# kekeliu-whu/Wildcat-SLAM

Measured on AMD Instinct MI355X. Metric: surfel-extract Mpts/s, higher is better.
Workload: dtype f64; 1 GPU; C2: 1M-pt single scan (G2 patch lattice, 999936 pts -> 31248 surfels) per GPU, voxel-grid + 3-level octree + per-cell 3x3 PCA; input = the reference's 48-byte hilti_ros::Point records, consumed in place; points_per_gpu=999936, surfels_per_gpu=31248, parallelism=sweep-per-gpu x1

## Files before the change

### wildcat-slam_amd/csrc/ctx.hip

```cpp
#include "ctx.h"

#include <cmath>
#include <cstring>
#include <mutex>

extern "C" const char *wc_version(void) { return "wildcat_hip 0.1 (gfx950)"; }

extern "C" int wc_device_count(void) {
  int n = 0;
  if (hipGetDeviceCount(&n) != hipSuccess) return 0;
  return n;
}

extern "C" void wc_params_default(wc_params *p) {
  std::memset(p, 0, sizeof(*p));
  p->voxel_size = 0.8f;
  p->max_layer = 2;
  p->min_points = 20;
  p->planer_threshold = 0.01f;
  p->min_plane_likeness = 0.1;
  p->cluster_gap = 0.05;
  p->cluster_min_points = 20;
  p->center_scale = 1.0;
  p->angular_scale = 5.0 * M_PI / 180.0;
// ... 37 lines not shown
    {"no_bucket_sort", "WC_NO_BUCKET_SORT", &wc_dev_opts::no_bucket_sort, true},
    {"ex_sync", "WC_EX_SYNC", &wc_dev_opts::ex_sync, true},
    {"match_pair_serial", "WC_MATCH_PAIR_SERIAL", &wc_dev_opts::match_pair_serial, true},
    {"lm_dense", "WC_LM_DENSE", &wc_dev_opts::lm_dense, true},
    {"lm_one_collective", "WC_LM_ONE_COLLECTIVE", &wc_dev_opts::lm_one_collective, true},
    {"lm_side_stream", "WC_LM_SIDE_STREAM", &wc_dev_opts::lm_side_stream, false},
    {"lm_dense_radius", "WC_LM_DENSE_RADIUS", &wc_dev_opts::lm_dense_radius, false},
    {"lm_radius0", "WC_LM_RADIUS0", &wc_dev_opts::lm_radius0, false},
};
}

namespace {
struct DevPool {
  hipMemPool_t pool = nullptr;
  int refs = 0;
};
std::mutex g_pool_mu;
DevPool g_pools[64];
}
hipMemPool_t wc_pool_acquire(int device) {
  if (device < 0 || device >= 64) return nullptr;
  std::lock_guard<std::mutex> lk(g_pool_mu);
  DevPool &d = g_pools[device];
  if (!d.pool) {
    int supported = 0;
    if (hipDeviceGetAttribute(&supported, hipDeviceAttributeMemoryPoolsSupported, device) != hipSuccess || !supported) {
      (void)hipGetLastError();
      return nullptr;
    }
    hipMemPoolProps props;
    std::memset(&props, 0, sizeof(props));
    props.allocType = hipMemAllocationTypePinned;
    props.handleTypes = hipMemHandleTypeNone;
    props.location.type = hipMemLocationTypeDevice;
    props.location.id = device;
    hipMemPool_t p = nullptr;
    if (hipMemPoolCreate(&p, &props) != hipSuccess || !p) {
      (void)hipGetLastError();
      return nullptr;
    }
    uint64_t keep = ~0ull;
    if (hipMemPoolSetAttribute(p, hipMemPoolAttrReleaseThreshold, &keep) != hipSuccess) (void)hipGetLastError();
    d.pool = p;
  }
  ++d.refs;
  return d.pool;
}
void wc_pool_release(int device, hipMemPool_t pool) {
  if (!pool || device < 0 || device >= 64) return;
  std::lock_guard<std::mutex> lk(g_pool_mu);
  DevPool &d = g_pools[device];
  if (d.pool == pool && --d.refs == 0) {
    (void)hipMemPoolDestroy(d.pool);
    d.pool = nullptr;
  }
}

extern "C" int wc_ctx_create(const wc_params *params, int device, wc_ctx **out) {
  if (!out) return WC_ERR_ARG;
  *out = nullptr;
  int n = 0;
  if (hipGetDeviceCount(&n) != hipSuccess || n <= 0 || device < 0 || device >= n) return WC_ERR_NOGPU;
  wc_ctx *ctx = new wc_ctx;
  ctx->device = device;
  if (params)
    ctx->P = *params;
  else
    wc_params_default(&ctx->P);
  int rc = check_params(ctx, &ctx->P);
  if (rc != WC_OK) {
    delete ctx;
    return rc;
  }
  int prev_dev = -1;
  (void)hipGetDevice(&prev_dev);
  struct Restore {
    int d;
    ~Restore() {
      if (d >= 0) (void)hipSetDevice(d);
    }
  } restore{prev_dev};
  if (hipSetDevice(device) != hipSuccess || hipStreamCreateWithFlags(&ctx->own_stream, hipStreamNonBlocking) != hipSuccess ||
      hipEventCreate(&ctx->ev0) != hipSuccess || hipEventCreate(&ctx->ev1) != hipSuccess ||
      hipHostMalloc((void **)&ctx->h_status, 128 * sizeof(uint32_t)) != hipSuccess ||
      hipHostMalloc((void **)&ctx->h_mail, (64 + 4096) * sizeof(double)) != hipSuccess) {
    delete ctx;
    return WC_ERR_HIP;
  }
  ctx->stream = ctx->own_stream;
  {
    void *dp = nullptr;
    if (hipHostGetDevicePointer(&dp, ctx->h_status, 0) == hipSuccess) ctx->h_status_dev = (uint32_t *)dp;
    for (int q = 0; q < 128; ++q) ctx->h_status[q] = 0;
  }
  for (wc_buf &b : ctx->b_route) b.plain = true;
  ctx->b_status.plain = true;
  ctx->pool = wc_pool_acquire(device);
  ctx->pool_ok = ctx->pool != nullptr;
#ifdef WC_DEV_KNOBS
  for (const DevOpt &o : kDevOpts)
    if (const char *v = getenv(o.env)) ctx->dev.*(o.field) = o.flag_only ? 1 : atoi(v);
#endif
  *out = ctx;
  return WC_OK;
}

extern "C" int wc_ctx_set_dev_option(wc_ctx *ctx, const char *name, int value) {
  if (!ctx || !name) return wc_fail(ctx, WC_ERR_ARG, "%s: null or out-of-range argument", __func__);
  for (const DevOpt &o : kDevOpts)
    if (strcmp(o.name, name) == 0) {
      ctx->dev.*(o.field) = value;
      ctx->ex.fx_backoff = ctx->ex.fx_skip_calls = 0;
      if (ctx->aux) ctx->aux->dev = ctx->dev;
      for (wc_ctx *sub : ctx->batch_subs) sub->dev = ctx->dev, sub->ex.fx_backoff = sub->ex.fx_skip_calls = 0;
      return WC_OK;
    }
  return wc_fail(ctx, WC_ERR_ARG, "wc_ctx_set_dev_option: unknown option '%s'", name);
}

void wc_window_free(wc_ctx *ctx);
extern "C" int wc_comm_rccl_destroy(wc_ctx *ctx);

extern "C" void wc_ctx_destroy(wc_ctx *ctx) {
  wc_dev_guard dg_(ctx);
  if (!ctx) return;
  (void)hipSetDevice(ctx->device);
  (void)hipStreamSynchronize(ctx->stream);
  if (ctx->pair_worker && ctx->pair_worker_free) ctx->pair_worker_free(ctx->pair_worker);
  ctx->pair_worker = nullptr;
  if (ctx->aux) {
    wc_ctx_destroy(ctx->aux);
    ctx->aux = nullptr;
  }
  if (ctx->ev_aux) (void)hipEventDestroy(ctx->ev_aux);
  if (ctx->ev_pair) (void)hipEventDestroy(ctx->ev_pair);
  for (hipEvent_t e : ctx->ev_knn)
    if (e) (void)hipEventDestroy(e);
  (void)wc_comm_rccl_destroy(ctx);
  wc_window_free(ctx);
  wc_buf *all[] = {&ctx->b_keys[0],      &ctx->b_keys[1],     &ctx->b_vals[0],     &ctx->b_vals[1],      &ctx->b_sorttmp,
                   &ctx->b_slots,        &ctx->b_slot_ids,    &ctx->b_slot_keys[0], &ctx->b_slot_keys[1], &ctx->b_slot_idx[0],
                   &ctx->b_slot_idx[1],  &ctx->b_cand,        &ctx->b_cand_meta,   &ctx->b_status,
                   &ctx->b_ex_ctrl};
  for (wc_buf *b : all) wc_buf_release(ctx, *b);
  for (wc_buf &b : ctx->b_misc) wc_buf_release(ctx, b);
  for (wc_buf &b : ctx->b_route) wc_buf_release(ctx, b);
  wc_buf_release(ctx, ctx->b_batch);
  for (wc_buf &b : ctx->b_kd) wc_buf_release(ctx, b);
  wc_buf_release(ctx, ctx->b_match_half);
  for (wc_ctx *sub : ctx->batch_subs) wc_ctx_destroy(sub);
  ctx->batch_subs.clear();
  for (wc_buf &b : ctx->b_fx) wc_buf_release(ctx, b);
  if (ctx->h_status) (void)hipHostFree(ctx->h_status);
  if (ctx->h_mail) (void)hipHostFree(ctx->h_mail);
  if (ctx->h_stage) (void)hipHostFree(ctx->h_stage);
  wc_buf_release(ctx, ctx->b_stage);
  (void)hipStreamSynchronize(ctx->stream);
  if (ctx->ev0) (void)hipEventDestroy(ctx->ev0);
  if (ctx->ev1) (void)hipEventDestroy(ctx->ev1);
  for (hipEvent_t e : ctx->ex_ev)
    if (e) (void)hipEventDestroy(e);
  if (ctx->own_stream) (void)hipStreamDestroy(ctx->own_stream);
  wc_pool_release(ctx->device, ctx->pool);
  delete ctx;
}

extern "C" const char *wc_last_error(const wc_ctx *ctx) { return ctx ? ctx->err.c_str() : "no context"; }
// ... 164 lines not shown
```

### wildcat-slam_amd/csrc/extract.hip

```cpp
#include <hip/hip_runtime.h>
#include <type_traits>

#include <chrono>
#include <cstdlib>
#include <cstring>
#include <rocprim/rocprim.hpp>

#include "ctx.h"
#include "dmath.h"

namespace {

constexpr int kMom = 11;
constexpr int kProdStride = 66;
constexpr unsigned kRootsGrid = 256 * 16;
constexpr unsigned kEmitGrid = 256 * 8;
constexpr unsigned kRoots2Grid = 256 * 4;
constexpr int kBuckets = 4096;
constexpr int kTile = 2048;
constexpr uint32_t kFlagKeyRange = 1u, kFlagSlotOverflow = 2u, kFlagTimeRange = 4u, kFlagBucketOverflow = 8u, kFlagSlotBinOverflow = 16u, kFlagLdsOverflow = 32u;

struct ExParams {
  double vs;
  float vs_f;
// ... 1120 lines not shown
      const uint32_t my_pos = (it + lane < it_end) ? A.heads[it + lane].pos : 0xFFFFFFFFu;
      unsigned long long live_mask = __ballot(my_pos != 0xFFFFFFFFu);
      while (live_mask) {
        uint32_t tslot = 0xFFFFFFFFu;
        for (int k = 0; k < NG; ++k) {
          if (!live_mask) break;
          const int bit = __ffsll((long long)live_mask) - 1;
          live_mask &= live_mask - 1;
          if (g == k) tslot = it + (uint32_t)bit;
        }
        do_roots(tslot);
      }
    }
  }
}

__global__ void __launch_bounds__(256) k_iota(uint32_t *v, uint64_t n) {
  const uint64_t i = (uint64_t)blockIdx.x * blockDim.x + threadIdx.x;
  if (i < n) v[i] = (uint32_t)i;
}

__global__ void __launch_bounds__(256) k_gather(const uint32_t *__restrict__ sorted_slot, const wc_surfel *__restrict__ slots,
                                               const wc_surfel_id *__restrict__ slot_ids, const uint32_t *status,
                                               wc_surfel *out, wc_surfel_id *out_ids, uint64_t cap) {
  if (status[1] & (kFlagBucketOverflow | kFlagKeyRange)) return;
  const uint64_t n = min((uint64_t)status[0], cap);
  const uint64_t i = (uint64_t)blockIdx.x * blockDim.x + threadIdx.x;
  const uint64_t rec = i / 10, part = i - rec * 10;
  if (rec >= n) return;
  const uint32_t s = sorted_slot[rec];
  if (part < 9) {
    const double2 *src = (const double2 *)(slots + s);
    double2 *dst = (double2 *)(out + rec);
    dst[part] = src[part];
  } else if (out_ids) {
    const uint4 *src = (const uint4 *)(slot_ids + s);
    uint4 *dst = (uint4 *)(out_ids + rec);
    *dst = *src;
  }
}

__device__ __forceinline__ bool surfel_id_less(const wc_surfel_id &a, const wc_surfel_id &b) {
  if (a.kx != b.kx) return a.kx < b.kx;
  if (a.ky != b.ky) return a.ky < b.ky;
  if (a.kz != b.kz) return a.kz < b.kz;
  return a.node < b.node;
}

__global__ void __launch_bounds__(256) k_fix_ties(const uint64_t *__restrict__ keys, uint32_t *idx, uint64_t n,
                                                 const wc_surfel_id *__restrict__ slot_ids) {
  const uint64_t i = (uint64_t)blockIdx.x * blockDim.x + threadIdx.x;
  if (i >= n) return;
  const uint64_t key = keys[i];
  if (key == ~0ull) return;
  if ((i > 0 && keys[i - 1] == key) || i + 1 >= n || keys[i + 1] != key) return;
  uint64_t e = i + 1;
  while (e < n && keys[e] == key) ++e;
  for (uint64_t a = i + 1; a < e; ++a) {
    const uint32_t v = idx[a];
    const wc_surfel_id vid = slot_ids[v];
    uint64_t b = a;
    while (b > i && surfel_id_less(vid, slot_ids[idx[b - 1]])) {
      idx[b] = idx[b - 1];
      --b;
    }
    idx[b] = v;
  }
}

constexpr int kSlotBinMax = 512;
struct SlotEmitArgs {
  const uint32_t *counts;
  const uint64_t *bins;
  uint32_t bin_cap;
  const wc_surfel *slots;
  const wc_surfel_id *slot_ids;
  uint32_t *status;
  wc_surfel *out;
  wc_surfel_id *out_ids;
  uint64_t cap;
  uint32_t *next_ctrl;
  uint32_t next_words;
};
__device__ __forceinline__ void slot_emit_body(const SlotEmitArgs &E, const uint32_t bid, const uint32_t nblk) {
  const uint32_t *__restrict__ counts = E.counts;
  const uint64_t *__restrict__ bins = E.bins;
  const uint32_t bin_cap = E.bin_cap;
  const wc_surfel *__restrict__ slots = E.slots;
  const wc_surfel_id *__restrict__ slot_ids = E.slot_ids;
  uint32_t *status = E.status;
  wc_surfel *out = E.out;
  wc_surfel_id *out_ids = E.out_ids;
  const uint64_t cap = E.cap;
  uint32_t *next_ctrl = E.next_ctrl;
  const uint32_t next_words = E.next_words;
  __shared__ uint64_t s_item[4][kSlotBinMax];
  if (next_ctrl) {
    const uint32_t i = bid * 256u + threadIdx.x;
    if (i < next_words) next_ctrl[i] = (i == 8u || i == 9u) ? status[i] : 0u;
  }
  __shared__ uint32_t s_sorted[4][kSlotBinMax];
  __shared__ uint32_t s_red[4];
  const int t = threadIdx.x, w = t >> 6, lane = t & 63;
  const uint32_t b0 = bid * 4u;
  static_assert(kBuckets / 4 <= 4 * 256, "four uint4 loads per thread cover the counts");
  const uint4 *c4 = (const uint4 *)counts;
  uint4 v[4];
#pragma unroll
  for (int k = 0; k < 4; ++k) {
    const uint32_t i = (uint32_t)t + 256u * k;
    v[k] = i < bid ? c4[i] : make_uint4(0u, 0u, 0u, 0u);
  }
  const uint4 own = c4[bid];
  const uint64_t *bin = bins + (size_t)(b0 + w) * bin_cap;
  const uint64_t first = (uint32_t)lane < bin_cap ? bin[lane] : 0ull;
  uint32_t part = 0;
#pragma unroll
  for (int k = 0; k < 4; ++k) part += v[k].x + v[k].y + v[k].z + v[k].w;
  for (int off = 32; off >= 1; off >>= 1) part += __shfl_xor(part, off);
  if (lane == 0) s_red[w] = part;
  __syncthreads();
  uint32_t base = s_red[0] + s_red[1] + s_red[2] + s_red[3];
  const uint32_t c0 = own.x, c1 = own.y, c2 = own.z, c3 = own.w;
  if (bid == nblk - 1 && t == 0) {
    status[0] = base + c0 + c1 + c2 + c3;
    uint32_t *hm = host_mailbox(status);
    if (hm) {
      hm[0] = base + c0 + c1 + c2 + c3;
      uint32_t queued = status[4];
      const uint32_t *fxc = counts + kBuckets;
      for (int j = 0; j < 16; ++j) queued += fxc[(16 + j) * 32];
      hm[4] = queued;
      hm[5] = status[5];
    }
  }
  base += (w > 0 ? c0 : 0u) + (w > 1 ? c1 : 0u) + (w > 2 ? c2 : 0u);
  const uint32_t c = w == 0 ? c0 : (w == 1 ? c1 : (w == 2 ? c2 : c3));
  if (c == 0) return;
  if (c > bin_cap) {
    if (lane == 0) raise_flag(status, kFlagSlotBinOverflow);
    return;
  }
  auto before = [&](uint64_t other, uint64_t mine) -> bool {
    if ((other >> 32) == (mine >> 32) && other != mine) {
      const double to = slots[(uint32_t)other].t, tm = slots[(uint32_t)mine].t;
      return to < tm || (to == tm && surfel_id_less(slot_ids[(uint32_t)other], slot_ids[(uint32_t)mine]));
    }
    return other < mine;
  };
  if (c <= 64u) {
    const uint32_t lo = (uint32_t)first, hi = (uint32_t)(first >> 32);
    uint32_t rank = 0;
    for (uint32_t j = 0; j < c; ++j) {
      const uint64_t other = ((uint64_t)(uint32_t)__builtin_amdgcn_readlane((int)hi, (int)j) << 32) | (uint32_t)__builtin_amdgcn_readlane((int)lo, (int)j);
      if ((uint32_t)lane < c) rank += before(other, first) ? 1u : 0u;
    }
    if ((uint32_t)lane < c) s_sorted[w][rank] = lo;
  } else {
    s_item[w][lane] = first;
    for (uint32_t i = lane + 64; i < c; i += 64) s_item[w][i] = bin[i];
    __builtin_amdgcn_wave_barrier();
    for (uint32_t i = lane; i < c; i += 64) {
      const uint64_t mine = s_item[w][i];
      uint32_t rank = 0;
      for (uint32_t j = 0; j < c; ++j) rank += before(s_item[w][j], mine) ? 1u : 0u;
      s_sorted[w][rank] = (uint32_t)mine;
    }
  }
  __builtin_amdgcn_wave_barrier();
  const int sub = lane / 10, piece = lane - sub * 10;
  if (sub >= 6) return;
  auto load = [&](uint32_t r, bool on) -> double2 {
    double2 d = make_double2(0.0, 0.0);
    if (!on) return d;
    const uint32_t sl = s_sorted[w][r];
    if (piece < 9)
      d = ((const double2 *)(slots + sl))[piece];
    else if (out_ids) {
      const uint4 q = *(const uint4 *)(slot_ids + sl);
      d = *(const double2 *)&q;
    }
    return d;
  };
  auto store = [&](uint32_t r, bool on, const double2 &d) {
    if (!on) return;
    const uint64_t o = (uint64_t)base + r;
    if (piece < 9)
      ((double2 *)(out + o))[piece] = d;
    else if (out_ids)
      *(double2 *)(out_ids + o) = d;
  };
  if (c <= 12u) {
    const uint32_t r = sub;
    const bool on0 = r < c && (uint64_t)base + r < cap, on1 = r + 6 < c && (uint64_t)base + r + 6 < cap;
    const double2 d0 = load(r, on0), d1 = load(r + 6, on1);
    store(r, on0, d0);
    store(r + 6, on1, d1);
    return;
  }
  for (uint32_t r = sub; r < c; r += 24) {
    bool on[4];
    double2 d[4];
#pragma unroll
    for (int q = 0; q < 4; ++q) {
      on[q] = r + 6u * q < c && (uint64_t)base + r + 6u * q < cap;
      d[q] = load(r + 6u * q, on[q]);
    }
#pragma unroll
    for (int q = 0; q < 4; ++q) store(r + 6u * q, on[q], d[q]);
  }
}

__global__ void __launch_bounds__(256) k_slot_emit(const uint32_t *__restrict__ counts, const uint64_t *__restrict__ bins, uint32_t bin_cap,
                                                  const wc_surfel *__restrict__ slots, const wc_surfel_id *__restrict__ slot_ids,
                                                  uint32_t *status, wc_surfel *out, wc_surfel_id *out_ids, uint64_t cap, uint32_t *next_ctrl,
                                                  uint32_t next_words) {
  const SlotEmitArgs E{counts, bins, bin_cap, slots, slot_ids, status, out, out_ids, cap, next_ctrl, next_words};
  slot_emit_body(E, blockIdx.x, gridDim.x);
}
__global__ void __launch_bounds__(256) k_slot_emit_b(const SlotEmitArgs *__restrict__ Es, int K) {
  const uint32_t per = kBuckets / 4;
  const uint32_t k = blockIdx.x / per;
  if ((int)k >= K) return;
  slot_emit_body(Es[k], blockIdx.x - k * per, per);
}


__device__ __forceinline__ uint32_t run_length(const unsigned long long *s_bits, uint32_t i, uint32_t cnt) {
  uint32_t w = (i + 1) >> 6;
  unsigned long long m = (w < kTile / 64) ? (s_bits[w] & (~0ull << ((i + 1) & 63))) : 0ull;
  while (m == 0ull && ++w < kTile / 64) m = s_bits[w];
  const uint32_t nxt = m ? (w * 64 + (uint32_t)__ffsll((long long)m) - 1) : cnt;
  return min(nxt, cnt) - i;
}

struct InitArgs {
  uint32_t *p[8];
  uint32_t nw[8];
  uint32_t val[8];
};
__global__ void __launch_bounds__(256) k_init(InitArgs I) {
  const uint32_t i = blockIdx.x * 256u + threadIdx.x;
#pragma unroll
  for (int r = 0; r < 8; ++r)
    if (i < I.nw[r]) I.p[r][i] = I.val[r];
}

constexpr int kRunThreads = 512;
__global__ void __launch_bounds__(kRunThreads) k_pt_runs(wc_points pts, double vs, uint64_t n, uint32_t *counts, uint64_t *bins,
                                                        uint32_t bin_cap, uint32_t *status) {
  __shared__ uint32_t s_key[kTile];
  __shared__ unsigned long long s_bits[kTile / 64];
  __shared__ uint32_t s_runs[kBuckets];
  __shared__ uint32_t s_pts[kBuckets];
  const int t = threadIdx.x;
  const uint64_t t0 = (uint64_t)blockIdx.x * kTile;
  const uint32_t cnt = (uint32_t)min((uint64_t)kTile, n - t0);
  double x0, y0, z0;
  load_xyz(pts, 0, x0, y0, z0);
  uint32_t key[kTile / kRunThreads];
#pragma unroll
  for (int j = 0; j < kTile / kRunThreads; ++j) {
    const uint32_t i = (uint32_t)j * kRunThreads + t;
    key[j] = 0;
    if (i < cnt) {
      double x, y, z;
      load_xyz(pts, t0 + i, x, y, z);
      int rx = vox(x, vs) - vox(x0, vs) + 512, ry = vox(y, vs) - vox(y0, vs) + 512, rz = vox(z, vs) - vox(z0, vs) + 512;
      if ((unsigned)rx >= 1024u || (unsigned)ry >= 1024u || (unsigned)rz >= 1024u) {
        raise_flag(status, kFlagKeyRange);
        rx = min(max(rx, 0), 1023), ry = min(max(ry, 0), 1023), rz = min(max(rz, 0), 1023);
      }
      key[j] = (uint32_t)rx | ((uint32_t)ry << 10) | ((uint32_t)rz << 20);
    }
  }
  for (int b = t; b < kBuckets; b += kRunThreads) {
    s_runs[b] = 0;
    s_pts[b] = 0;
  }
  if (t < kTile / 64) s_bits[t] = 0ull;
#pragma unroll
  for (int j = 0; j < kTile / kRunThreads; ++j) s_key[j * kRunThreads + t] = key[j];
  __syncthreads();
#pragma unroll
  for (int j = 0; j < kTile / kRunThreads; ++j) {
    const uint32_t i = (uint32_t)j * kRunThreads + t;
    const bool headp = i < cnt && (i == 0 || key[j] != s_key[i - 1]);
    const unsigned long long m = __ballot(headp);
    if ((t & 63) == 0) s_bits[i >> 6] = m;
  }
  __syncthreads();
  uint32_t rank[kTile / kRunThreads], len[kTile / kRunThreads];
#pragma unroll
  for (int j = 0; j < kTile / kRunThreads; ++j) {
    const uint32_t i = (uint32_t)j * kRunThreads + t;
    rank[j] = 0xFFFFFFFFu;
    if (i < cnt && ((s_bits[i >> 6] >> (i & 63)) & 1ull)) {
      const uint32_t d = key_digit(key[j]);
      len[j] = run_length(s_bits, i, cnt);
      rank[j] = atomicAdd(&s_runs[d], 1u);
      atomicAdd(&s_pts[d], len[j]);
    }
  }
  __syncthreads();
  for (int b = t; b < kBuckets; b += kRunThreads) {
    const uint32_t c = s_runs[b];
    if (c) {
// ... 53 lines not shown
    }
  } else {
    uint32_t N = 128;
    while (N < nb) N <<= 1;
    s_b[lane] = first;
    for (uint32_t i = lane + 64; i < N; i += 64) s_b[i] = (i < nb) ? bin[i] : ~0ull;
    __builtin_amdgcn_wave_barrier();
    for (uint32_t k = 2; k <= N; k <<= 1)
      for (uint32_t j = k >> 1; j > 0; j >>= 1) {
        for (uint32_t p = lane; p < N / 2; p += 64) {
          const uint32_t i = 2 * p - (p & (j - 1)), l = i + j;
          const uint64_t x = s_b[i], y = s_b[l];
          if ((x > y) == ((i & k) == 0)) {
            s_b[i] = y;
            s_b[l] = x;
          }
        }
        __builtin_amdgcn_wave_barrier();
      }
  }
  __builtin_amdgcn_wave_barrier();
  uint32_t carry = 0;
  for (uint32_t i0 = 0; i0 < nb; i0 += 64) {
    const uint32_t i = i0 + lane;
    const uint64_t c = (i < nb) ? s_b[i] : 0ull;
    const uint32_t l = (i < nb) ? comp_len(c) : 0u;
    uint32_t inc = l;
    for (int off = 1; off < 64; off <<= 1) {
      const uint32_t v = __shfl_up(inc, off);
      if (lane >= off) inc += v;
    }
    if (i < nb) {
      s_off[i] = carry + inc - l;
      bin[i] = c;
      run_off[(size_t)b * bin_cap + i] = carry + inc - l;
    }
    carry += __shfl(inc, 63);
  }
  __builtin_amdgcn_wave_barrier();
  uint32_t *s_list = (uint32_t *)s_a;
  uint32_t nlive = 0, next_head = nb;
  for (int i0 = (int)((nb + 63) / 64) * 64 - 64; i0 >= 0; i0 -= 64) {
    const uint32_t r = (uint32_t)i0 + lane;
    const bool in = r < nb;
    const uint32_t rest = in ? comp_rest(s_b[r]) : 0u;
    const bool head = in && (r == 0 || comp_rest(s_b[r - 1]) != rest);
    const unsigned long long hm = __ballot(head);
    const unsigned long long above = (lane == 63) ? 0ull : (hm >> (lane + 1));
    const uint32_t r2 = above ? r + (uint32_t)__ffsll((long long)above) : next_head;
    const uint32_t seg = (r2 < nb ? s_off[min(r2, nb - 1)] : total) - (in ? s_off[r] : 0u);
    const bool live = head && seg > (uint32_t)min_points;
    const unsigned long long lm = __ballot(live);
    if (live) s_list[nlive + (uint32_t)__popcll(lm & ((1ull << lane) - 1ull))] = r | (r2 << 16);
    nlive += (uint32_t)__popcll(lm);
    if (hm) next_head = (uint32_t)i0 + (uint32_t)__ffsll((long long)hm) - 1u;
  }
  if (lane == 0) s_live[w] = nlive;
  __syncthreads();
  const uint32_t pbase0 = s_red[0] + s_red[1] + s_red[2] + s_red[3];
  const uint32_t pbase = pbase0 + before;
  const uint32_t first_slot = pbase0 / (uint32_t)(min_points + 1);
  uint32_t lbase = 0;
  for (int j = 0; j < w; ++j) lbase += s_live[j];
  if (t == 0) {
    root_cnt[blockIdx.x] = s_live[0] + s_live[1] + s_live[2] + s_live[3];
    root_first[blockIdx.x] = first_slot;
  }
  for (uint32_t k = lane; k < nlive; k += 64) {
    const uint32_t r = s_list[k] & 0xFFFFu, r2 = s_list[k] >> 16;
    const uint32_t seg = (r2 < nb ? s_off[r2] : total) - s_off[r];
    head_slots[first_slot + lbase + k] = HeadRec{pbase + s_off[r], b * bin_cap + r, r2 - r, seg};
  }
}

constexpr uint32_t kPtBinMax = 1024;

inline uint32_t pt_bin_cap(uint64_t n) {
  uint32_t cap = 64;
  while (cap < kPtBinMax && (uint64_t)cap * kBuckets < 32 * n) cap *= 2;
  return cap;
}

constexpr uint32_t kCtrlStatus = 0, kCtrlCounts = 64, kCtrlRoots = kCtrlCounts + 2 * kBuckets, kCtrlBins = kCtrlRoots + 2 * (kBuckets / 4),
                   kCtrlFx = kCtrlBins + kBuckets, kCtrlWords = kCtrlFx + 4 * 16 * 32;

int clear_ctrl(wc_ctx *ctx) {
  WC_TRY(wc_ensure(ctx, ctx->b_ex_ctrl, kCtrlWords * 4));
  uint32_t *ctrl = (uint32_t *)ctx->b_ex_ctrl.p;
  InitArgs I{};
  void *dp = nullptr;
  if (hipHostGetDevicePointer(&dp, ctx->h_status, 0) != hipSuccess) dp = nullptr;
  const unsigned long long a = (unsigned long long)dp;
  I.p[0] = ctrl, I.nw[0] = 8, I.val[0] = 0u;
  I.p[1] = ctrl + 10, I.nw[1] = kCtrlRoots - 10, I.val[1] = 0u;
  I.p[2] = ctrl + 8, I.nw[2] = 1, I.val[2] = (uint32_t)a;
  I.p[3] = ctrl + 9, I.nw[3] = 1, I.val[3] = (uint32_t)(a >> 32);
  I.p[4] = ctrl + kCtrlBins, I.nw[4] = kBuckets + 4 * 16 * 32, I.val[4] = 0u;
  k_init<<<(kCtrlRoots + 255) / 256, 256, 0, ctx->stream>>>(I);
  WC_HIP(ctx, hipGetLastError());
  return WC_OK;
}

int point_sort_runs(wc_ctx *ctx, const wc_points &pts, double vs, HeadRec *head_slots, int min_points, uint32_t *status) {
  hipStream_t st = ctx->stream;
  const uint64_t n = pts.n;
  const uint32_t cap = pt_bin_cap(n);
  const uint32_t lds_cap = std::min(cap, std::max(64u, ctx->ex.lds_cap));
  WC_TRY(wc_ensure(ctx, ctx->b_misc[1], (uint64_t)kBuckets * cap * 8));
  WC_TRY(wc_ensure(ctx, ctx->b_misc[3], (uint64_t)kBuckets * cap * 4));
  uint32_t *counts = (uint32_t *)ctx->b_ex_ctrl.p + kCtrlCounts;
  const unsigned tiles = (unsigned)((n + kTile - 1) / kTile);
  const size_t lds = (size_t)4 * lds_cap * 20;
  if (!ctx->ex.bucket_attr_set) {
    WC_HIP(ctx, hipFuncSetAttribute((const void *)k_pt_bucket, hipFuncAttributeMaxDynamicSharedMemorySize, (int)(4 * kPtBinMax * 20)));
    ctx->ex.bucket_attr_set = true;
  }
  k_pt_runs<<<tiles, kRunThreads, 0, st>>>(pts, vs, n, counts, (uint64_t *)ctx->b_misc[1].p, cap, status);
  k_pt_bucket<<<kBuckets / 4, 256, lds, st>>>((uint64_t *)ctx->b_misc[1].p, cap, lds_cap, counts, (uint32_t *)ctx->b_misc[3].p, head_slots,
                                             counts + 2 * kBuckets, counts + 2 * kBuckets + kBuckets / 4, min_points, status);
  WC_HIP(ctx, hipGetLastError());
  return WC_OK;
}

template <typename K>
int sort_pairs(wc_ctx *ctx, K *kin, K *kout, uint32_t *vin, uint32_t *vout, size_t n, unsigned end_bit) {
  using cfg = rocprim::radix_sort_config<rocprim::default_config, rocprim::default_config, rocprim::default_config, 0>;
  size_t tmp = 0;
  WC_HIP(ctx, rocprim::radix_sort_pairs<cfg>(nullptr, tmp, kin, kout, vin, vout, n, 0u, end_bit, ctx->stream));
  WC_TRY(wc_ensure(ctx, ctx->b_sorttmp, tmp));
  tmp = ctx->b_sorttmp.cap;
  WC_HIP(ctx, rocprim::radix_sort_pairs<cfg>(ctx->b_sorttmp.p, tmp, kin, kout, vin, vout, n, 0u, end_bit, ctx->stream));
  return WC_OK;
}

#include "extract_fast.inc"
#include "extract_split.inc"

int fx_ensure_zero(wc_ctx *ctx, wc_buf &b, size_t bytes) {
  if (bytes <= b.cap) return WC_OK;
  WC_TRY(wc_ensure(ctx, b, bytes));
  WC_HIP(ctx, hipMemsetAsync(b.p, 0, b.cap, ctx->stream));
  return WC_OK;
}

bool fx_applicable(const wc_ctx *ctx, uint64_t n, double t_lo, double t_hi) {
  const wc_params &P = ctx->P;
  if (P.exact_sums || ctx->dev.exact_sums) return false;
  if (n < 64 || !(P.voxel_size > 0.0f) || P.voxel_size >= 0.99f) return false;
  if (!(P.cluster_gap > 1e-6) || !(t_hi > t_lo)) return false;
  if ((t_hi - t_lo) / (P.cluster_gap * 0.999) >= 1048000.0) return false;
  return true;
}

int fx_tail(wc_ctx *ctx, bool layer2);

int run_pipeline_fast(wc_ctx *ctx, const wc_points &pts, double t_lo, double t_hi, wc_surfel *d_out, wc_surfel_id *d_ids, uint64_t cap) {
  const wc_params &P = ctx->P;
  const uint64_t n = pts.n;
  hipStream_t st = ctx->stream;
  FxArgs A;
  std::memset(&A, 0, sizeof(A));
  ExParams &E = A.P;
  E.vs = (double)P.voxel_size, E.vs_f = P.voxel_size, E.max_layer = P.max_layer, E.min_points = P.min_points;
  E.thr = (double)P.planer_threshold, E.min_like = P.min_plane_likeness;
  for (int i = 0; i < 3; ++i) E.view[i] = P.view_point[i];
  E.gap = P.cluster_gap, E.cluster_min = P.cluster_min_points;
  E.t_lo_bits = ordered_bits_host(t_lo);
// ... 57 lines not shown
    ctx->ex.fx_dirty = false;
  }
  WC_TRY(wc_ensure(ctx, ctx->b_fx[5], (size_t)2 * kCtrlWords * 4));
  if (!ctx->ex.fx_ctrl_ready) {
    WC_HIP(ctx, hipMemsetAsync(ctx->b_fx[5].p, 0, (size_t)2 * kCtrlWords * 4, st));
    void *dp = nullptr;
    if (hipHostGetDevicePointer(&dp, ctx->h_status, 0) != hipSuccess) dp = nullptr;
    const unsigned long long a = (unsigned long long)dp;
    const uint32_t addr[2] = {(uint32_t)a, (uint32_t)(a >> 32)};
    for (int b = 0; b < 2; ++b)
      WC_HIP(ctx, hipMemcpyAsync((uint32_t *)ctx->b_fx[5].p + (size_t)b * kCtrlWords + 8, addr, 8, hipMemcpyHostToDevice, st));
    WC_HIP(ctx, hipStreamSynchronize(st));
    ctx->ex.fx_ctrl_ready = true;
    ctx->ex.fx_parity = 0;
  }
  uint32_t *ctrl = (uint32_t *)ctx->b_fx[5].p + (size_t)ctx->ex.fx_parity * kCtrlWords;
  for (int q = 0; q < 64; ++q) ctx->h_status[q] = 0;
  A.rkey = (uint32_t *)ctx->b_fx[0].p, A.rlist = (uint32_t *)ctx->b_fx[1].p;
  A.blk = (unsigned long long *)ctx->b_fx[2].p, A.blk2 = (unsigned long long *)ctx->b_fx[3].p;
  A.rec = (unsigned long long *)ctx->b_fx[4].p;
  A.jobs = (unsigned long long *)ctx->b_fx[6].p;
  A.status = ctrl + kCtrlStatus;
  A.cnt = ctrl + kCtrlFx;
  A.slots = (wc_surfel *)ctx->b_slots.p, A.slot_ids = (wc_surfel_id *)ctx->b_slot_ids.p;
  A.slots_per = (uint32_t)std::min<uint64_t>(total_slots / kFxSub, 0x7FFFFFFFu);
  A.slot_counts = ctrl + kCtrlBins;
  A.slot_bins = (uint64_t *)ctx->b_slot_keys[1].p;
  A.slot_bin_cap = bin_cap;
  auto mark = [&](int i) {
    if (ctx->ex_prof && (ctx->ex_prof_mode != 2 || i == 1 || i == 5)) (void)hipEventRecord(ctx->ex_ev[i], st);
  };
  mark(0);
  mark(1);
  static const bool dbg = wc_log_env("WC_FX_DEBUG");
  auto dbg_sync = [&](const char *what) {
    if (!dbg) return;
    fprintf(stderr, "[fx] %s ...", what);
    const hipError_t e = hipStreamSynchronize(st);
    uint32_t w[64], c[4 * 16 * 32];
    (void)hipMemcpy(w, A.status, sizeof(w), hipMemcpyDeviceToHost);
    (void)hipMemcpy(c, A.cnt, sizeof(c), hipMemcpyDeviceToHost);
    uint32_t r = 0, q = 0, sl = 0, sp = 0;
    for (int j = 0; j < 16; ++j) r += c[j * 32], q += c[(16 + j) * 32], sl += c[(32 + j) * 32], sp += c[(48 + j) * 32];
    fprintf(stderr, " %s flags=%u roots=%u nodes2=%u slots=%u spill=%u\n", hipGetErrorString(e), w[1], r, q, sl, sp);
  };
  if (dbg) fprintf(stderr, "[fx] n=%llu tiles=%u mr_per=%u mq_per=%u tr=%u slots_per=%u bin_cap=%u\n", (unsigned long long)n, tiles, A.mr_per, A.mq_per, tr, A.slots_per, bin_cap);
  if (ctx->ex.batch_defer) {
    static_assert(sizeof(FxArgs) <= sizeof(ctx->ex.roots_args), "ctx.h: roots_args too small");
    std::memcpy(ctx->ex.roots_args, &A, sizeof(A));
    ctx->ex.total_slots = total_slots;
    ctx->ex.bin_cap = bin_cap;
    ctx->ex.fast_slots = true;
    ctx->ex.tail = &fx_tail;
    ctx->ex.d_out = d_out, ctx->ex.d_ids = d_ids, ctx->ex.cap = cap;
    ctx->ex.layer2_done = P.max_layer >= 2 && ctx->ex.last_splits > 0;
    ctx->ex.fx_tiles = tiles, ctx->ex.fx_ngrid = std::max(64u, ngrid / 8u);
    ctx->ex.deferred = true;
    return WC_OK;
  }
  k_fx_acc<1><<<tiles, kFxThreads, 0, st>>>(A);
  dbg_sync("k_fx_acc<1>");
  mark(2);
  if (ctx->ex.fx_long_lists) k_fx_merge<1><<<std::min<unsigned>(ngrid * 2u, 8192u), 128, 0, st>>>(A);
  if (ctx->ex.fx_split) {
    k_fx_walk<1><<<ngrid, 64, 0, st>>>(A);
    dbg_sync("k_fx_walk<1>");
    k_fx_test<1><<<ngrid, 64, 0, st>>>(A);
  } else {
    k_fx_nodes<1><<<ngrid, 64, 0, st>>>(A);
  }
  dbg_sync("k_fx_nodes<1>");
  mark(3);
  static_assert(sizeof(FxArgs) <= sizeof(ctx->ex.roots_args), "ctx.h: roots_args too small");
  std::memcpy(ctx->ex.roots_args, &A, sizeof(A));
  ctx->ex.total_slots = total_slots;
  ctx->ex.bin_cap = bin_cap;
  ctx->ex.fast_slots = true;
  ctx->ex.tail = &fx_tail;
  ctx->ex.d_out = d_out, ctx->ex.d_ids = d_ids, ctx->ex.cap = cap;
  return fx_tail(ctx, P.max_layer >= 2 && ctx->ex.last_splits > 0);
}

constexpr int kMailTicket = 120;
__global__ void k_ex_ticket(uint32_t *host_word, uint32_t ticket) {
  __hip_atomic_store(host_word, ticket, __ATOMIC_RELEASE, __HIP_MEMORY_SCOPE_SYSTEM);
}

int fx_tail(wc_ctx *ctx, bool layer2) {
  hipStream_t st = ctx->stream;
  FxArgs A;
  std::memcpy(&A, ctx->ex.roots_args, sizeof(A));
  auto mark = [&](int i) {
    if (ctx->ex_prof && (ctx->ex_prof_mode != 2 || i == 1 || i == 5)) (void)hipEventRecord(ctx->ex_ev[i], st);
  };
  if (layer2) {
    const unsigned tiles = (unsigned)((A.pts.n + kFxTile - 1) / kFxTile);
    k_fx_acc<2><<<tiles, kFxThreads, 0, st>>>(A);
    const unsigned ngrid = std::min<unsigned>(256 * 16, std::max<unsigned>(64, (unsigned)(A.pts.n / 256)));
    if (ctx->ex.fx_long_lists2) k_fx_merge<2><<<std::min(8192u, std::max(64u, ctx->ex.last_splits)), 128, 0, st>>>(A);
    const unsigned g2 = std::min(std::min(256u * 8u, ngrid), std::max(64u, ctx->ex.last_splits));
    if (ctx->ex.fx_split) {
      k_fx_walk<2><<<g2, 64, 0, st>>>(A);
      k_fx_test<2><<<g2, 64, 0, st>>>(A);
    } else {
      k_fx_nodes<2><<<g2, 64, 0, st>>>(A);
    }
  }
  ctx->ex.layer2_done = layer2;
  mark(4);
  uint32_t *next_ctrl = (uint32_t *)ctx->b_fx[5].p + (size_t)(ctx->ex.fx_parity ^ 1) * kCtrlWords;
  static_assert(kCtrlWords <= (kBuckets / 4) * 256, "k_slot_emit's grid covers the control block");
  k_slot_emit<<<kBuckets / 4, 256, 0, st>>>(A.slot_counts, A.slot_bins, ctx->ex.bin_cap, (const wc_surfel *)ctx->b_slots.p,
                                           (const wc_surfel_id *)ctx->b_slot_ids.p, A.status, ctx->ex.d_out, ctx->ex.d_ids, ctx->ex.cap, next_ctrl,
                                           kCtrlWords);
  mark(5);
  ctx->ex.ticket = 0;
  if (ctx->h_status_dev && !ctx->ex_prof && !ctx->dev.ex_sync) {
    if (++ctx->ex.ticket_seq == 0u) ++ctx->ex.ticket_seq;
    ctx->ex.ticket = ctx->ex.ticket_seq;
    k_ex_ticket<<<1, 1, 0, st>>>(ctx->h_status_dev + kMailTicket, ctx->ex.ticket);
  }
  static const bool fx_dbg = wc_log_env("WC_FX_DEBUG");
  if (fx_dbg) fprintf(stderr, "[fx] k_slot_emit (layer2=%d) ... %s\n", (int)layer2, hipGetErrorString(hipStreamSynchronize(st)));
  WC_HIP(ctx, hipGetLastError());
  return WC_OK;
}

template <typename K, bool RUNS>
int pipeline_tail(wc_ctx *ctx, bool layer2) {
  hipStream_t st = ctx->stream;
  RootsArgs A;
  memcpy(&A, ctx->ex.roots_args, sizeof(A));
  uint32_t *status = A.status;
  wc_surfel *d_out = ctx->ex.d_out;
  wc_surfel_id *d_ids = ctx->ex.d_ids;
  const uint64_t cap = ctx->ex.cap, total_slots = ctx->ex.total_slots;
  auto mark = [&](int i) {
    if (ctx->ex_prof && (ctx->ex_prof_mode != 2 || i == 1 || i == 5)) (void)hipEventRecord(ctx->ex_ev[i], st);
  };
  if (layer2) {
    const unsigned grid2 = std::min(kRoots2Grid, std::max(64u, ctx->ex.last_splits));
    if constexpr (RUNS) {
      if (ctx->ex.unordered)
        k_roots_banks<K, 2, true><<<grid2, 64, 0, st>>>(A, (const K *)ctx->b_keys[1].p);
      else
        k_roots<K, 2, true><<<grid2, 64, 0, st>>>(A, (const K *)ctx->b_keys[1].p);
    } else {
      k_roots_banks<K, 2, false><<<grid2, 64, 0, st>>>(A, (const K *)ctx->b_keys[1].p);
    }
  }
  ctx->ex.layer2_done = layer2;
  mark(4);
  if (ctx->ex.fast_slots) {
    k_slot_emit<<<kBuckets / 4, 256, 0, st>>>((const uint32_t *)ctx->b_ex_ctrl.p + kCtrlBins, A.slot_bins, ctx->ex.bin_cap, (const wc_surfel *)ctx->b_slots.p,
                                             (const wc_surfel_id *)ctx->b_slot_ids.p, status, d_out, d_ids, cap, nullptr, 0u);
  } else {
    k_iota<<<(unsigned)((total_slots + 255) / 256), 256, 0, st>>>((uint32_t *)ctx->b_slot_idx[0].p, total_slots);
    WC_TRY(sort_pairs<uint64_t>(ctx, (uint64_t *)ctx->b_slot_keys[0].p, (uint64_t *)ctx->b_slot_keys[1].p,
                                (uint32_t *)ctx->b_slot_idx[0].p, (uint32_t *)ctx->b_slot_idx[1].p, total_slots,
                                ctx->ex.slot_end_bit));
    k_fix_ties<<<(unsigned)((total_slots + 255) / 256), 256, 0, st>>>((const uint64_t *)ctx->b_slot_keys[1].p, (uint32_t *)ctx->b_slot_idx[1].p,
                                                                     total_slots, (const wc_surfel_id *)ctx->b_slot_ids.p);
    const uint64_t gth = std::min<uint64_t>(total_slots, cap) * 10;
    if (gth)
      k_gather<<<(unsigned)((gth + 255) / 256), 256, 0, st>>>((const uint32_t *)ctx->b_slot_idx[1].p, (const wc_surfel *)ctx->b_slots.p,
                                                             (const wc_surfel_id *)ctx->b_slot_ids.p, status, d_out, d_ids, cap);
  }
  mark(5);
  if (!ctx->ex.fast_slots) WC_HIP(ctx, hipMemcpyAsync(ctx->h_status, status, 32, hipMemcpyDeviceToHost, st));
  WC_HIP(ctx, hipGetLastError());
  return WC_OK;
}

template <typename K>
int run_pipeline(wc_ctx *ctx, const wc_points &pts, double t_lo, double t_hi, wc_surfel *d_out, wc_surfel_id *d_ids,
                 uint64_t cap, bool fast, bool fast_order) {
  const wc_params &P = ctx->P;
  const uint64_t n = pts.n;
  hipStream_t st = ctx->stream;
  ExParams E;
  E.vs = (double)P.voxel_size;
  E.vs_f = P.voxel_size;
  E.max_layer = P.max_layer;
  E.min_points = P.min_points;
  E.thr = (double)P.planer_threshold;
  E.min_like = P.min_plane_likeness;
  for (int i = 0; i < 3; ++i) E.view[i] = P.view_point[i];
  E.gap = P.cluster_gap;
  E.cluster_min = P.cluster_min_points;
  E.t_lo_bits = ordered_bits_host(t_lo);
  E.dbg = ctx->dev.debug_skip;
  E.merge_min = ctx->dev.fx_merge_min;
  const uint64_t span = ordered_bits_host(t_hi) - E.t_lo_bits;
  E.t_span_bits = span;
  unsigned tbits = 1;
  while (tbits < 64 && (span >> tbits)) ++tbits;
  const unsigned slot_end_bit = tbits >= 63 ? 64 : tbits + 1;

  const uint64_t total_slots = (n * (uint64_t)(P.max_layer + 1)) / (uint64_t)P.cluster_min_points + 1;
  WC_TRY(wc_ensure(ctx, ctx->b_keys[0], n * sizeof(K)));
  WC_TRY(wc_ensure(ctx, ctx->b_keys[1], n * sizeof(K)));
  WC_TRY(wc_ensure(ctx, ctx->b_vals[0], n * 4));
  WC_TRY(wc_ensure(ctx, ctx->b_vals[1], n * 4));
  WC_TRY(wc_ensure(ctx, ctx->b_cand, total_slots * kMom * 8));
  WC_TRY(wc_ensure(ctx, ctx->b_cand_meta, total_slots * 4));
  WC_TRY(wc_ensure(ctx, ctx->b_slots, total_slots * sizeof(wc_surfel)));
  WC_TRY(wc_ensure(ctx, ctx->b_slot_ids, total_slots * sizeof(wc_surfel_id)));
  WC_TRY(wc_ensure(ctx, ctx->b_slot_keys[0], total_slots * 8));
  WC_TRY(wc_ensure(ctx, ctx->b_slot_keys[1], total_slots * 8));
  WC_TRY(wc_ensure(ctx, ctx->b_slot_idx[0], total_slots * 4));
  WC_TRY(wc_ensure(ctx, ctx->b_slot_idx[1], total_slots * 4));
  WC_TRY(wc_ensure(ctx, ctx->b_misc[0], (n / (uint64_t)(P.min_points + 1) + 2) * sizeof(HeadRec)));
  const bool precleared = ctx->ex.precleared && ctx->b_ex_ctrl.p;
  ctx->ex.precleared = false;
  if (!precleared) WC_TRY(clear_ctrl(ctx));
  for (int q = 0; q < 16; ++q) ctx->h_status[q] = 0;
  uint32_t *status = (uint32_t *)ctx->b_ex_ctrl.p + kCtrlStatus;

  auto mark = [&](int i) {
    if (ctx->ex_prof && (ctx->ex_prof_mode != 2 || i == 1 || i == 5)) (void)hipEventRecord(ctx->ex_ev[i], st);
  };
  mark(0);
  const bool fast_slots = fast_order && tbits <= 31 && total_slots < (1ull << 31);
  uint32_t bin_cap = 64;
  while (bin_cap < kSlotBinMax && (uint64_t)bin_cap * kBuckets < 2 * total_slots) bin_cap *= 2;
  const unsigned g256 = (unsigned)((n + 255) / 256);
  const bool fast_pts = fast && sizeof(K) == 4;
  if (fast_pts || fast_slots) {
    WC_TRY(wc_ensure(ctx, ctx->b_slot_keys[1], (uint64_t)kBuckets * bin_cap * 8));
  }
  const uint32_t nslots = (uint32_t)(n / (uint64_t)(P.min_points + 1) + 1);
  if (!fast_slots || !fast_pts) {
    InitArgs I{};
    int r = 0;
    auto fill = [&](void *p, uint64_t words, uint32_t v) { I.p[r] = (uint32_t *)p, I.nw[r] = (uint32_t)words, I.val[r] = v, ++r; };
    if (!fast_slots) fill(ctx->b_slot_keys[0].p, total_slots * 2, 0xFFFFFFFFu);
    if (!fast_pts) fill(ctx->b_misc[0].p, (uint64_t)nslots * 4, 0xFFFFFFFFu);
    uint32_t mx = 0;
// ... 395 lines not shown
```

Baseline: 21650 Mpts/s.

## Fold completion ticket into slot-emit via last-block arrival counters

Removes the separate single-thread ticket kernel launched after k_slot_emit. Each workgroup now counts itself on hierarchical arrival counters, and the last one publishes the host-visible ticket. Output stores go through buffer-resource b128 stores, and mailbox writes become system-scope atomics so the host can poll completion without an extra kernel launch. The cost is extra atomics per workgroup, a coherent host allocation for the status words, and added memory-ordering complexity: the publishes are relaxed atomics placed after a vmcnt wait.

Result: no change. 21370 Mpts/s, median of 2 (-1.3%).

```diff
diff --git a/wildcat-slam_amd/csrc/ctx.hip b/wildcat-slam_amd/csrc/ctx.hip
--- a/wildcat-slam_amd/csrc/ctx.hip
+++ b/wildcat-slam_amd/csrc/ctx.hip
@@ -143,7 +143,7 @@
   } restore{prev_dev};
   if (hipSetDevice(device) != hipSuccess || hipStreamCreateWithFlags(&ctx->own_stream, hipStreamNonBlocking) != hipSuccess ||
       hipEventCreate(&ctx->ev0) != hipSuccess || hipEventCreate(&ctx->ev1) != hipSuccess ||
-      hipHostMalloc((void **)&ctx->h_status, 128 * sizeof(uint32_t)) != hipSuccess ||
+      hipHostMalloc((void **)&ctx->h_status, 128 * sizeof(uint32_t), hipHostMallocCoherent) != hipSuccess ||
       hipHostMalloc((void **)&ctx->h_mail, (64 + 4096) * sizeof(double)) != hipSuccess) {
     delete ctx;
     return WC_ERR_HIP;
diff --git a/wildcat-slam_amd/csrc/extract.hip b/wildcat-slam_amd/csrc/extract.hip
--- a/wildcat-slam_amd/csrc/extract.hip
+++ b/wildcat-slam_amd/csrc/extract.hip
@@ -1226,9 +1226,32 @@
   uint32_t *next_ctrl;
   uint32_t next_words;
 };
-__device__ __forceinline__ void slot_emit_body(const SlotEmitArgs &E, const uint32_t bid, const uint32_t nblk) {
-  const uint32_t *__restrict__ counts = E.counts;
-  const uint64_t *__restrict__ bins = E.bins;
+constexpr uint32_t kArriveSubs = 32, kArriveWords = (kArriveSubs + 1) * 32;
+static_assert((kBuckets / 4) % kArriveSubs == 0, "every sub-counter counts the same number of workgroups");
+typedef __attribute__((address_space(1))) uint32_t gu32;
+struct SlotPublish {
+  uint32_t *arrive;
+  uint32_t *ticket_word;
+  uint32_t ticket;
+};
+
+__device__ __forceinline__ __amdgpu_buffer_rsrc_t wave_rsrc(const void *p) {
+  const unsigned long long a = (unsigned long long)p;
+  const unsigned long long u = ((unsigned long long)(uint32_t)__builtin_amdgcn_readfirstlane((int)(uint32_t)(a >> 32)) << 32) |
+                               (uint32_t)__builtin_amdgcn_readfirstlane((int)(uint32_t)a);
+  return __builtin_amdgcn_make_buffer_rsrc((void *)u, (short)0, 0x7FFFFFFF, 0x00020000);
+}
+__device__ __forceinline__ void store_wt16(__amdgpu_buffer_rsrc_t r, uint32_t off, const double2 &d) {
+  typedef unsigned u32x4 __attribute__((ext_vector_type(4)));
+  u32x4 q;
+  __builtin_memcpy(&q, &d, 16);
+  __builtin_amdgcn_raw_buffer_store_b128(q, r, (int)off, 0, 16);
+}
+
+template <bool PUB>
+__device__ __forceinline__ void slot_emit_bucket(const SlotEmitArgs &E, uint32_t base, const uint32_t c, const uint64_t *bin,
+                                                 const uint64_t first, uint64_t (&s_item)[4][kSlotBinMax],
+                                                 uint32_t (&s_sorted)[4][kSlotBinMax]) {
   const uint32_t bin_cap = E.bin_cap;
   const wc_surfel *__restrict__ slots = E.slots;
   const wc_surfel_id *__restrict__ slot_ids = E.slot_ids;
@@ -1236,6 +1259,105 @@
   wc_surfel *out = E.out;
   wc_surfel_id *out_ids = E.out_ids;
   const uint64_t cap = E.cap;
+  const int t = threadIdx.x, w = t >> 6, lane = t & 63;
+  if (c == 0) return;
+  if (c > bin_cap) {
+    if (lane == 0) {
+      if constexpr (PUB) {
+        atomicOr(&status[1], kFlagSlotBinOverflow);
+        if (uint32_t *hm = host_mailbox(status))
+          __hip_atomic_store((gu32 *)hm + 8 + (__ffs((int)kFlagSlotBinOverflow) - 1), 1u, __ATOMIC_RELAXED, __HIP_MEMORY_SCOPE_SYSTEM);
+      } else {
+        raise_flag(status, kFlagSlotBinOverflow);
+      }
+    }
+    return;
+  }
+  auto before = [&](uint64_t other, uint64_t mine) -> bool {
+    if ((other >> 32) == (mine >> 32) && other != mine) {
+      const double to = slots[(uint32_t)other].t, tm = slots[(uint32_t)mine].t;
+      return to < tm || (to == tm && surfel_id_less(slot_ids[(uint32_t)other], slot_ids[(uint32_t)mine]));
+    }
+    return other < mine;
+  };
+  if (c <= 64u) {
+    const uint32_t lo = (uint32_t)first, hi = (uint32_t)(first >> 32);
+    uint32_t rank = 0;
+    for (uint32_t j = 0; j < c; ++j) {
+      const uint64_t other = ((uint64_t)(uint32_t)__builtin_amdgcn_readlane((int)hi, (int)j) << 32) | (uint32_t)__builtin_amdgcn_readlane((int)lo, (int)j);
+      if ((uint32_t)lane < c) rank += before(other, first) ? 1u : 0u;
+    }
+    if ((uint32_t)lane < c) s_sorted[w][rank] = lo;
+  } else {
+    s_item[w][lane] = first;
+    for (uint32_t i = lane + 64; i < c; i += 64) s_item[w][i] = bin[i];
+    __builtin_amdgcn_wave_barrier();
+    for (uint32_t i = lane; i < c; i += 64) {
+      const uint64_t mine = s_item[w][i];
+      uint32_t rank = 0;
+      for (uint32_t j = 0; j < c; ++j) rank += before(s_item[w][j], mine) ? 1u : 0u;
+      s_sorted[w][rank] = (uint32_t)mine;
+    }
+  }
+  __builtin_amdgcn_wave_barrier();
+  const int sub = lane / 10, piece = lane - sub * 10;
+  if (sub >= 6) return;
+  auto load = [&](uint32_t r, bool on) -> double2 {
+    double2 d = make_double2(0.0, 0.0);
+    if (!on) return d;
+    const uint32_t sl = s_sorted[w][r];
+    if (piece < 9)
+      d = ((const double2 *)(slots + sl))[piece];
+    else if (out_ids) {
+      const uint4 q = *(const uint4 *)(slot_ids + sl);
+      d = *(const double2 *)&q;
+    }
+    return d;
+  };
+  __amdgpu_buffer_rsrc_t r_out, r_ids;
+  if constexpr (PUB) r_out = wave_rsrc(out + base), r_ids = wave_rsrc(out_ids ? out_ids + base : nullptr);
+  auto store = [&](uint32_t r, bool on, const double2 &d) {
+    if (!on) return;
+    if constexpr (PUB) {
+      if (piece < 9)
+        store_wt16(r_out, r * (uint32_t)sizeof(wc_surfel) + (uint32_t)piece * 16u, d);
+      else if (out_ids)
+        store_wt16(r_ids, r * (uint32_t)sizeof(wc_surfel_id), d);
+      return;
+    }
+    const uint64_t o = (uint64_t)base + r;
+    if (piece < 9)
+      ((double2 *)(out + o))[piece] = d;
+    else if (out_ids)
+      *(double2 *)(out_ids + o) = d;
+  };
+  if (c <= 12u) {
+    const uint32_t r = sub;
+    const bool on0 = r < c && (uint64_t)base + r < cap, on1 = r + 6 < c && (uint64_t)base + r + 6 < cap;
+    const double2 d0 = load(r, on0), d1 = load(r + 6, on1);
+    store(r, on0, d0);
+    store(r + 6, on1, d1);
+    return;
+  }
+  for (uint32_t r = sub; r < c; r += 24) {
+    bool on[4];
+    double2 d[4];
+#pragma unroll
+    for (int q = 0; q < 4; ++q) {
+      on[q] = r + 6u * q < c && (uint64_t)base + r + 6u * q < cap;
+      d[q] = load(r + 6u * q, on[q]);
+    }
+#pragma unroll
+    for (int q = 0; q < 4; ++q) store(r + 6u * q, on[q], d[q]);
+  }
+}
+
+template <bool PUB>
+__device__ __forceinline__ void slot_emit_body(const SlotEmitArgs &E, const uint32_t bid, const uint32_t nblk, const SlotPublish &Pb) {
+  const uint32_t *__restrict__ counts = E.counts;
+  const uint64_t *__restrict__ bins = E.bins;
+  const uint32_t bin_cap = E.bin_cap;
+  uint32_t *status = E.status;
   uint32_t *next_ctrl = E.next_ctrl;
   const uint32_t next_words = E.next_words;
   __shared__ uint64_t s_item[4][kSlotBinMax];
@@ -1270,103 +1392,51 @@
     status[0] = base + c0 + c1 + c2 + c3;
     uint32_t *hm = host_mailbox(status);
     if (hm) {
-      hm[0] = base + c0 + c1 + c2 + c3;
       uint32_t queued = status[4];
       const uint32_t *fxc = counts + kBuckets;
       for (int j = 0; j < 16; ++j) queued += fxc[(16 + j) * 32];
-      hm[4] = queued;
-      hm[5] = status[5];
+      const uint32_t runs = status[5];
+      if constexpr (PUB) {
+        __hip_atomic_store((gu32 *)hm + 0, base + c0 + c1 + c2 + c3, __ATOMIC_RELAXED, __HIP_MEMORY_SCOPE_SYSTEM);
+        __hip_atomic_store((gu32 *)hm + 4, queued, __ATOMIC_RELAXED, __HIP_MEMORY_SCOPE_SYSTEM);
+        __hip_atomic_store((gu32 *)hm + 5, runs, __ATOMIC_RELAXED, __HIP_MEMORY_SCOPE_SYSTEM);
+      } else {
+        hm[0] = base + c0 + c1 + c2 + c3;
+        hm[4] = queued;
+        hm[5] = runs;
+      }
     }
   }
   base += (w > 0 ? c0 : 0u) + (w > 1 ? c1 : 0u) + (w > 2 ? c2 : 0u);
   const uint32_t c = w == 0 ? c0 : (w == 1 ? c1 : (w == 2 ? c2 : c3));
-  if (c == 0) return;
-  if (c > bin_cap) {
-    if (lane == 0) raise_flag(status, kFlagSlotBinOverflow);
-    return;
-  }
-  auto before = [&](uint64_t other, uint64_t mine) -> bool {
-    if ((other >> 32) == (mine >> 32) && other != mine) {
-      const double to = slots[(uint32_t)other].t, tm = slots[(uint32_t)mine].t;
-      return to < tm || (to == tm && surfel_id_less(slot_ids[(uint32_t)other], slot_ids[(uint32_t)mine]));
-    }
-    return other < mine;
-  };
-  if (c <= 64u) {
-    const uint32_t lo = (uint32_t)first, hi = (uint32_t)(first >> 32);
-    uint32_t rank = 0;
-    for (uint32_t j = 0; j < c; ++j) {
-      const uint64_t other = ((uint64_t)(uint32_t)__builtin_amdgcn_readlane((int)hi, (int)j) << 32) | (uint32_t)__builtin_amdgcn_readlane((int)lo, (int)j);
-      if ((uint32_t)lane < c) rank += before(other, first) ? 1u : 0u;
-    }
-    if ((uint32_t)lane < c) s_sorted[w][rank] = lo;
-  } else {
-    s_item[w][lane] = first;
-    for (uint32_t i = lane + 64; i < c; i += 64) s_item[w][i] = bin[i];
-    __builtin_amdgcn_wave_barrier();
-    for (uint32_t i = lane; i < c; i += 64) {
-      const uint64_t mine = s_item[w][i];
-      uint32_t rank = 0;
-      for (uint32_t j = 0; j < c; ++j) rank += before(s_item[w][j], mine) ? 1u : 0u;
-      s_sorted[w][rank] = (uint32_t)mine;
-    }
-  }
-  __builtin_amdgcn_wave_barrier();
-  const int sub = lane / 10, piece = lane - sub * 10;
-  if (sub >= 6) return;
-  auto load = [&](uint32_t r, bool on) -> double2 {
-    double2 d = make_double2(0.0, 0.0);
-    if (!on) return d;
-    const uint32_t sl = s_sorted[w][r];
-    if (piece < 9)
-      d = ((const double2 *)(slots + sl))[piece];
-    else if (out_ids) {
-      const uint4 q = *(const uint4 *)(slot_ids + sl);
-      d = *(const double2 *)&q;
-    }
-    return d;
-  };
-  auto store = [&](uint32_t r, bool on, const double2 &d) {
-    if (!on) return;
-    const uint64_t o = (uint64_t)base + r;
-    if (piece < 9)
-      ((double2 *)(out + o))[piece] = d;
-    else if (out_ids)
-      *(double2 *)(out_ids + o) = d;
-  };
-  if (c <= 12u) {
-    const uint32_t r = sub;
-    const bool on0 = r < c && (uint64_t)base + r < cap, on1 = r + 6 < c && (uint64_t)base + r + 6 < cap;
-    const double2 d0 = load(r, on0), d1 = load(r + 6, on1);
-    store(r, on0, d0);
-    store(r + 6, on1, d1);
-    return;
-  }
-  for (uint32_t r = sub; r < c; r += 24) {
-    bool on[4];
-    double2 d[4];
-#pragma unroll
-    for (int q = 0; q < 4; ++q) {
-      on[q] = r + 6u * q < c && (uint64_t)base + r + 6u * q < cap;
-      d[q] = load(r + 6u * q, on[q]);
-    }
-#pragma unroll
-    for (int q = 0; q < 4; ++q) store(r + 6u * q, on[q], d[q]);
-  }
-}
-
+  slot_emit_bucket<PUB>(E, base, c, bin, first, s_item, s_sorted);
+  if constexpr (PUB) {
+    asm volatile("s_waitcnt vmcnt(0)" ::: "memory");
+    __syncthreads();
+    if (t != 0) return;
+    uint32_t *sub = Pb.arrive + (bid % kArriveSubs) * 32u;
+    if (__hip_atomic_fetch_add(sub, 1u, __ATOMIC_RELAXED, __HIP_MEMORY_SCOPE_AGENT) + 1u != nblk / kArriveSubs) return;
+    __hip_atomic_store(sub, 0u, __ATOMIC_RELAXED, __HIP_MEMORY_SCOPE_AGENT);
+    uint32_t *top = Pb.arrive + kArriveSubs * 32u;
+    if (__hip_atomic_fetch_add(top, 1u, __ATOMIC_RELAXED, __HIP_MEMORY_SCOPE_AGENT) + 1u != kArriveSubs) return;
+    __hip_atomic_store(top, 0u, __ATOMIC_RELAXED, __HIP_MEMORY_SCOPE_AGENT);
+    __hip_atomic_store((gu32 *)Pb.ticket_word, Pb.ticket, __ATOMIC_RELAXED, __HIP_MEMORY_SCOPE_SYSTEM);
+  }
+}
+
+template <bool PUB>
 __global__ void __launch_bounds__(256) k_slot_emit(const uint32_t *__restrict__ counts, const uint64_t *__restrict__ bins, uint32_t bin_cap,
                                                   const wc_surfel *__restrict__ slots, const wc_surfel_id *__restrict__ slot_ids,
                                                   uint32_t *status, wc_surfel *out, wc_surfel_id *out_ids, uint64_t cap, uint32_t *next_ctrl,
-                                                  uint32_t next_words) {
+                                                  uint32_t next_words, SlotPublish Pb) {
   const SlotEmitArgs E{counts, bins, bin_cap, slots, slot_ids, status, out, out_ids, cap, next_ctrl, next_words};
-  slot_emit_body(E, blockIdx.x, gridDim.x);
+  slot_emit_body<PUB>(E, blockIdx.x, gridDim.x, Pb);
 }
 __global__ void __launch_bounds__(256) k_slot_emit_b(const SlotEmitArgs *__restrict__ Es, int K) {
   const uint32_t per = kBuckets / 4;
   const uint32_t k = blockIdx.x / per;
   if ((int)k >= K) return;
-  slot_emit_body(Es[k], blockIdx.x - k * per, per);
+  slot_emit_body<false>(Es[k], blockIdx.x - k * per, per, SlotPublish{});
 }
 
 
@@ -1586,7 +1656,9 @@
 }
 
 constexpr uint32_t kCtrlStatus = 0, kCtrlCounts = 64, kCtrlRoots = kCtrlCounts + 2 * kBuckets, kCtrlBins = kCtrlRoots + 2 * (kBuckets / 4),
-                   kCtrlFx = kCtrlBins + kBuckets, kCtrlWords = kCtrlFx + 4 * 16 * 32;
+                   kCtrlFx = kCtrlBins + kBuckets, kCtrlArrive = kCtrlFx + 4 * 16 * 32,
+                   kCtrlWords = kCtrlArrive + kArriveWords;
+static_assert(kCtrlArrive % 32 == 0 && kCtrlWords % 32 == 0, "arrival counters on lines of their own, in both control blocks");
 
 int clear_ctrl(wc_ctx *ctx) {
   WC_TRY(wc_ensure(ctx, ctx->b_ex_ctrl, kCtrlWords * 4));
@@ -1810,9 +1882,6 @@
 }
 
 constexpr int kMailTicket = 120;
-__global__ void k_ex_ticket(uint32_t *host_word, uint32_t ticket) {
-  __hip_atomic_store(host_word, ticket, __ATOMIC_RELEASE, __HIP_MEMORY_SCOPE_SYSTEM);
-}
 
 int fx_tail(wc_ctx *ctx, bool layer2) {
   hipStream_t st = ctx->stream;
@@ -1836,18 +1905,23 @@
   }
   ctx->ex.layer2_done = layer2;
   mark(4);
+  uint32_t *ctrl = (uint32_t *)ctx->b_fx[5].p + (size_t)ctx->ex.fx_parity * kCtrlWords;
   uint32_t *next_ctrl = (uint32_t *)ctx->b_fx[5].p + (size_t)(ctx->ex.fx_parity ^ 1) * kCtrlWords;
   static_assert(kCtrlWords <= (kBuckets / 4) * 256, "k_slot_emit's grid covers the control block");
-  k_slot_emit<<<kBuckets / 4, 256, 0, st>>>(A.slot_counts, A.slot_bins, ctx->ex.bin_cap, (const wc_surfel *)ctx->b_slots.p,
-                                           (const wc_surfel_id *)ctx->b_slot_ids.p, A.status, ctx->ex.d_out, ctx->ex.d_ids, ctx->ex.cap, next_ctrl,
-                                           kCtrlWords);
-  mark(5);
   ctx->ex.ticket = 0;
   if (ctx->h_status_dev && !ctx->ex_prof && !ctx->dev.ex_sync) {
     if (++ctx->ex.ticket_seq == 0u) ++ctx->ex.ticket_seq;
     ctx->ex.ticket = ctx->ex.ticket_seq;
-    k_ex_ticket<<<1, 1, 0, st>>>(ctx->h_status_dev + kMailTicket, ctx->ex.ticket);
-  }
+    const SlotPublish Pb{ctrl + kCtrlArrive, ctx->h_status_dev + kMailTicket, ctx->ex.ticket};
+    k_slot_emit<true><<<kBuckets / 4, 256, 0, st>>>(A.slot_counts, A.slot_bins, ctx->ex.bin_cap, (const wc_surfel *)ctx->b_slots.p,
+                                                   (const wc_surfel_id *)ctx->b_slot_ids.p, A.status, ctx->ex.d_out, ctx->ex.d_ids, ctx->ex.cap,
+                                                   next_ctrl, kCtrlWords, Pb);
+  } else {
+    k_slot_emit<false><<<kBuckets / 4, 256, 0, st>>>(A.slot_counts, A.slot_bins, ctx->ex.bin_cap, (const wc_surfel *)ctx->b_slots.p,
+                                                    (const wc_surfel_id *)ctx->b_slot_ids.p, A.status, ctx->ex.d_out, ctx->ex.d_ids, ctx->ex.cap,
+                                                    next_ctrl, kCtrlWords, SlotPublish{});
+  }
+  mark(5);
   static const bool fx_dbg = wc_log_env("WC_FX_DEBUG");
   if (fx_dbg) fprintf(stderr, "[fx] k_slot_emit (layer2=%d) ... %s\n", (int)layer2, hipGetErrorString(hipStreamSynchronize(st)));
   WC_HIP(ctx, hipGetLastError());
@@ -1880,8 +1954,9 @@
   ctx->ex.layer2_done = layer2;
   mark(4);
   if (ctx->ex.fast_slots) {
-    k_slot_emit<<<kBuckets / 4, 256, 0, st>>>((const uint32_t *)ctx->b_ex_ctrl.p + kCtrlBins, A.slot_bins, ctx->ex.bin_cap, (const wc_surfel *)ctx->b_slots.p,
-                                             (const wc_surfel_id *)ctx->b_slot_ids.p, status, d_out, d_ids, cap, nullptr, 0u);
+    k_slot_emit<false><<<kBuckets / 4, 256, 0, st>>>((const uint32_t *)ctx->b_ex_ctrl.p + kCtrlBins, A.slot_bins, ctx->ex.bin_cap,
+                                                    (const wc_surfel *)ctx->b_slots.p, (const wc_surfel_id *)ctx->b_slot_ids.p, status, d_out, d_ids,
+                                                    cap, nullptr, 0u, SlotPublish{});
   } else {
     k_iota<<<(unsigned)((total_slots + 255) / 256), 256, 0, st>>>((uint32_t *)ctx->b_slot_idx[0].p, total_slots);
     WC_TRY(sort_pairs<uint64_t>(ctx, (uint64_t *)ctx->b_slot_keys[0].p, (uint64_t *)ctx->b_slot_keys[1].p,
```
